# luoyetx/JDA

Measured on AMD Instinct MI355X. Metric: candidate windows/sec, 640x480 batch (jdaDetect hot path); FDDB images/sec in config.fddb_images_per_s, higher is better.
Workload: dtype f32

## Files before the change

jda_amd/csrc/finish_common.h:

```cpp
#pragma once
#include "kernels_common.h"

namespace jda {

namespace {

template <typename Real>
struct Stp { Real scale, r00, r01, r10, r11; };

template <typename Real>
__device__ __forceinline__ void stp_apply(const Stp<Real>& p, Real x, Real y, Real* x2, Real* y2) {
  *x2 = p.scale * (p.r00 * x + p.r01 * y);
  *y2 = p.scale * (p.r10 * x + p.r11 * y);
}

__device__ __forceinline__ Stp<double> stp_calc(const double* s1, const double* __restrict__ s2, int L,
                                                double* t1, double* t2) {
  double x1c = 0., y1c = 0., x2c = 0., y2c = 0.;
  for (int i = 0; i < L; i++) { x1c += s1[2 * i]; y1c += s1[2 * i + 1]; x2c += s2[2 * i]; y2c += s2[2 * i + 1]; }
  x1c /= (double)L; y1c /= (double)L; x2c /= (double)L; y2c /= (double)L;
  for (int i = 0; i < L; i++) {
    t1[2 * i] = s1[2 * i] - x1c; t1[2 * i + 1] = s1[2 * i + 1] - y1c;
    t2[2 * i] = s2[2 * i] - x2c; t2[2 * i + 1] = s2[2 * i + 1] - y2c;
  }
// ... 97 lines not shown
      const double r = sqrt(2.0);
      v1->ox = (int)((double)x / r); v1->oy = (int)((double)y / r); v1->pw = (int)((double)wn / r);
      v2->ox = x / 2; v2->oy = y / 2; v2->pw = wn / 2;
    }
  }
}

__device__ __forceinline__ void load_window_tile(const uint8_t* __restrict__ wbase, int W, int win, uint8_t* tile,
                                                 int tpitch, int lane, int nthreads = 64, const Bc& bc = Bc()) {
  const int dpr = tpitch >> 2;
  const float inv = 1.0f / (float)dpr;
  const int total = win * dpr;
  uint32_t* t32 = (uint32_t*)tile;
  for (int idx = lane; idx < total; idx += nthreads) {
    const int y = (int)(((float)idx + 0.5f) * inv);
    const int j = idx - y * dpr;
    const uint8_t* p = wbase + (size_t)y * W + 4 * j;
    const unsigned sft = (unsigned)((uintptr_t)p & 3u);
    const uint32_t* q = (const uint32_t*)(p - sft);
#ifdef JDA_BOUNDS_CHECK
    if ((long long)(uintptr_t)q + 4 <= bc.lo || (long long)(uintptr_t)q >= bc.hi) jda_bc_fail(kBcWindowTileLoad, __LINE__);
    if ((int)sft + min(4, win - 4 * j) > 4 && ((long long)(uintptr_t)(q + 1) + 4 <= bc.lo || (long long)(uintptr_t)(q + 1) >= bc.hi)) jda_bc_fail(kBcWindowTileLoad, __LINE__);
    JDA_BC(Bc(0, (long long)tpitch * win), (long long)idx * 4, 4, kBcWindowTileLoad);
#endif
    const uint32_t lo = q[0];
    uint32_t hi = 0;
    if ((int)sft + min(4, win - 4 * j) > 4) hi = q[1];
    t32[idx] = __builtin_amdgcn_alignbyte(hi, lo, sft);
  }
}

}

template <typename DL, int G, bool MULTI, bool ST, bool TILE = false>
__device__ __forceinline__ void walk_carts(const NodeOff<typename DL::Real>* __restrict__ stage_off,
                                           const uint2* __restrict__ stage_meta, int K, const int* k,
                                           int depth, int node_n, const typename DL::Real* sh, int win,
                                           const View& v0, const View& v1, const View& v2,
                                           const Stp<typename DL::Real>& stp, bool apply_st, int* leaf,
                                           const uint8_t* tile = nullptr, int tpitch = 0,
                                           const typename DL::Node* __restrict__ stage_deep = nullptr, int split = 1 << 20) {
  int node[G];
#pragma unroll
  for (int g = 0; g < G; g++) node[g] = 0;
  const int levels = depth - 1;
  const int shallow = min(levels, split);
  for (int d = 0; d < shallow; d++) {
    const unsigned first = (1u << d) - 1u, lvl = (unsigned)K * first - first;
    typename DL::Node nd[G];
#pragma unroll
    for (int g = 0; g < G; g++) {
      const unsigned o = lvl + ((unsigned)k[g] << d) + (unsigned)node[g];
      const NodeOff<typename DL::Real> f = stage_off[o];
      const uint2 mt = stage_meta[o];
      nd[g].o1x = f.o1x; nd[g].o1y = f.o1y; nd[g].o2x = f.o2x; nd[g].o2y = f.o2y;
      nd[g].lm1x2 = (int)(mt.x & 0x7fffu); nd[g].lm2x2 = (int)((mt.x >> 15) & 0x7fffu); nd[g].scale = (int)(mt.x >> 30);
      nd[g].th = (int)mt.y;
    }
    int feat[G];
#pragma unroll
    for (int g = 0; g < G; g++) feat[g] = node_feature<DL, MULTI, ST, TILE>(nd[g], sh, win, v0, v1, v2, stp, apply_st, tile, tpitch);
#pragma unroll
    for (int g = 0; g < G; g++) node[g] = 2 * node[g] + (feat[g] <= nd[g].th ? 1 : 2);
  }
  for (int d = shallow; d < levels; d++) {
    typename DL::Node nd[G];
#pragma unroll
    for (int g = 0; g < G; g++)
      nd[g] = stage_deep[lm_deep_index((unsigned)k[g], (unsigned)d, (unsigned)node[g], (unsigned)levels, (unsigned)split)];
    int feat[G];
#pragma unroll
    for (int g = 0; g < G; g++) feat[g] = node_feature<DL, MULTI, ST, TILE>(nd[g], sh, win, v0, v1, v2, stp, apply_st, tile, tpitch);
#pragma unroll
    for (int g = 0; g < G; g++) node[g] = 2 * node[g] + (feat[g] <= nd[g].th ? 1 : 2);
  }
#pragma unroll
  for (int g = 0; g < G; g++) leaf[g] = node[g] - node_n;
}

template <int G, bool TILE>
__device__ __forceinline__ void walk_carts_s0(const S0Node* __restrict__ tbl, int K, const int* k, int depth, int node_n,
                                              const uint8_t* __restrict__ pix, int pitch, int* leaf, const Bc& bc = Bc()) {
  int node[G];
#pragma unroll
  for (int g = 0; g < G; g++) node[g] = 0;
  for (int d = 0; d < depth - 1; d++) {
    const unsigned first = (1u << d) - 1u, lvl = (unsigned)K * first - first;
    S0Node r[G];
#pragma unroll
    for (int g = 0; g < G; g++) r[g] = tbl[lvl + ((unsigned)k[g] << d) + (unsigned)node[g]];
    int pa[G], pb[G];
#pragma unroll
    for (int g = 0; g < G; g++) {
      const unsigned p1 = r[g].lo & 0x3fffffu, p2 = __builtin_amdgcn_alignbit(r[g].hi, r[g].lo, 22) & 0x3fffffu;
#ifdef JDA_BOUNDS_CHECK
      if (TILE) { JDA_BC(bc, __umul24(p1 >> 11, (unsigned)pitch) + (p1 & 0x7ffu), 1, kBcFinishTile); JDA_BC(bc, __umul24(p2 >> 11, (unsigned)pitch) + (p2 & 0x7ffu), 1, kBcFinishTile); }
      else { JDA_BC_ADDR(bc, pix + __umul24(p1 >> 11, (unsigned)pitch) + (p1 & 0x7ffu), 1, kBcFinishPix); JDA_BC_ADDR(bc, pix + __umul24(p2 >> 11, (unsigned)pitch) + (p2 & 0x7ffu), 1, kBcFinishPix); }
#endif
      pa[g] = pix[__umul24(p1 >> 11, (unsigned)pitch) + (p1 & 0x7ffu)];
      pb[g] = pix[__umul24(p2 >> 11, (unsigned)pitch) + (p2 & 0x7ffu)];
    }
#pragma unroll
    for (int g = 0; g < G; g++) node[g] = 2 * node[g] + (pa[g] - pb[g] <= (int)((r[g].hi >> 12) & 0x3ffu) - 256 ? 1 : 2);
  }
#pragma unroll
  for (int g = 0; g < G; g++) leaf[g] = node[g] - node_n;
}


}
```

jda_amd/csrc/host.h:

```cpp
#pragma once
#include <hip/hip_runtime_api.h>

#include <algorithm>
#include <atomic>
#include <chrono>
#include <cmath>
#include <cstdio>
#include <cstdlib>
#include <cstring>
#include <condition_variable>
#include <exception>
#include <functional>
#include <memory>
#include <map>
#include <mutex>
#include <numeric>
#include <new>
#include <stdexcept>
#include <string>
#include <thread>
#include <tuple>
#include <vector>

#include "../../include/jda.h"
// ... 35 lines not shown
  catch (...) {}
  try { fail(std::string(fn) + ": " + what); }
  catch (...) { std::fprintf(stderr, "libjda: %s: %s\n", fn, what); }
  if (sync_device) { (void)hipDeviceSynchronize(); (void)hipGetLastError(); }
}
#define JDA_ABI_CATCH(ret) catch (...) { jda::abi_exception(__func__, false); return ret; }
#define JDA_ABI_CATCH_SYNC(ret) catch (...) { jda::abi_exception(__func__, true); return ret; }
#define JDA_ABI_CATCH_VOID catch (...) { jda::abi_exception(__func__, false); }

constexpr int kLdsGranule = 1280, kLdsGranules = 128;
inline int lds_wgs_per_cu(long long lds_bytes) { return lds_bytes <= 0 ? kLdsGranules : (int)(kLdsGranules / ((lds_bytes + kLdsGranule - 1) / kLdsGranule)); }
inline int lds_bytes_for_wgs(int wgs_per_cu) { return (kLdsGranules / std::max(1, wgs_per_cu)) * kLdsGranule; }

inline long long env_ll(const char* name, long long dflt) {
  const char* v = std::getenv(name);
  return v && *v ? std::atoll(v) : dflt;
}

#define JDA_KNOBS(X)                                                                                   \
  X(handoff, "JDA_HANDOFF", 128)             \
  X(no_fast_scan, "JDA_NO_FAST_SCAN", 0)                                                               \
  X(plan_cache, "JDA_PLAN_CACHE", 64)                                 \
  X(dense, "JDA_DENSE", 1)                                                \
  X(merge_blocks, "JDA_MERGE_BLOCKS", 2048)  \
  X(side_small, "JDA_SIDE_SMALL", 1)                                                                   \
  X(side_stream, "JDA_SIDE_STREAM", 1)                                                                 \
  X(wide_max, "JDA_WIDE_MAX", 1024)          \
  X(wide_conc, "JDA_WIDE_CONC", 1)           \
  X(h2d_stream, "JDA_H2D_STREAM", 1)         \
  X(h2d_min_bytes, "JDA_H2D_MIN_BYTES", 8 << 20)  \
  X(kernel_d2h, "JDA_KERNEL_D2H", 1)         \
  X(filter0, "JDA_FILTER0", 1)               \
  X(fin_carry, "JDA_FIN_CARRY", 1)           \
  X(predict, "JDA_PREDICT", 1)               \
  X(debug_times, "JDA_DEBUG_TIMES", 0)                                                                 \
  X(test_wpf_scale, "JDA_TEST_WPF_SCALE", 1)              \
  X(test_throw, "JDA_TEST_THROW", 0)         \
  X(lanes, "JDA_LANES", 2)                                 \
  X(lanes_min_windows, "JDA_LANES_MIN_WINDOWS", 2000000)                                               \
  X(workspace_mb, "JDA_WORKSPACE_MB", 24 * 1024)                                                       \
  X(ws_bound, "JDA_WS_BOUND", 1)             \
  X(ws_factor_pct, "JDA_WS_FACTOR_PCT", 400)  \
  X(ws_min_entries, "JDA_WS_MIN_ENTRIES", 65536)  \
  X(ragged_chunk_windows, "JDA_RAGGED_CHUNK_WINDOWS", 4000000)  \
  X(ragged_chunk_windows_cpp, "JDA_RAGGED_CHUNK_WINDOWS_CPP", 8000000)  \
  X(mine_chunk_windows, "JDA_MINE_CHUNK_WINDOWS", 4194304)  \
  X(lbf_lds_kb, "JDA_LBF_LDS_KB", 160)       \
  X(ragged_chunk_min_windows, "JDA_RAGGED_CHUNK_MIN_WINDOWS", 1500000)  \
  X(ragged_split, "JDA_RAGGED_SPLIT", 3)     \
  X(ragged_single_windows, "JDA_RAGGED_SINGLE_WINDOWS", 5000000)  \
  X(hwq_place, "JDA_HWQ_PLACE", 1)           \
  X(max_lanes, "JDA_MAX_LANES", 16)          \
  X(lane_idle_calls, "JDA_LANE_IDLE_CALLS", 256)  \
  X(device_post, "JDA_DEVICE_POST", 1)       \
  X(device_post_min_frames, "JDA_DEVICE_POST_MIN_FRAMES", 16)  \
  X(w_pad, "JDA_W_PAD", 1)                   \
  X(lm_deep, "JDA_LM_DEEP", 1)               \
  X(w_stream_mb, "JDA_W_STREAM_MB", 8)       \
  X(scan_p, "JDA_SCAN_P", 1)                 \
  X(scan_p_ragged, "JDA_SCAN_P_RAGGED", 1)   \
  X(scan_p_block, "JDA_SCAN_P_BLOCK", 768)                               \
  X(scan_p_slots, "JDA_SCAN_P_SLOTS", 5)     \
  X(scan_p_b0, "JDA_SCAN_P_B0", 32)                \
  X(scan_p_b1, "JDA_SCAN_P_B1", 64)                                                                    \
  X(scan_p_b2, "JDA_SCAN_P_B2", 0)                                                                     \
  X(scan_p_b3, "JDA_SCAN_P_B3", 0)                                                                     \
// ... 455 lines not shown
```

jda_amd/csrc/k_finish.hip:

```cpp
#include "finish_common.h"

#ifndef FIN_ROW_BATCH
#define FIN_ROW_BATCH 0
#endif

namespace jda {


template <typename DL, bool TRACE, int kG, bool MULTI, bool ST, bool STREAM = false>
__global__ __launch_bounds__(64) void k_finish(const DevPlan* __restrict__ plan, DevModelT<typename DL::Real> m,
                                               WorkT<typename DL::Real> w, int multi_i, float inv_sqrt2,
                                               int t_begin, int t_end, int apply_th, typename DL::Real final_th,
                                               const S0Node* __restrict__ s0_table, int tile_win, int survivors) {
  using Real = typename DL::Real;
  constexpr bool kCpp = sizeof(Real) == 8;
  extern __shared__ __attribute__((aligned(16))) unsigned char lds[];
  const int lane = threadIdx.x;
  const int T = m.T, K = m.K, node_n = m.node_n, leaf_n = m.leaf_n, dim = m.dim, w_pitch = m.w_pitch;
  const int dim_pad = (dim + 1) & ~1;
  Real* sh = (Real*)lds;
  uint32_t* lbf = (uint32_t*)(sh + dim_pad);
  int* stage_cnt = (int*)(lbf + ((K + 3) & ~3));
  Real* st_tmp = (Real*)(stage_cnt + kMaxStages);
  uint8_t* tile = lds + (((size_t)((unsigned char*)(st_tmp + (ST ? 2 * dim_pad + 8 : 0)) - lds) + 15) & ~(size_t)15);
  constexpr bool multi = MULTI;
  (void)multi_i;
  if (lane < kMaxStages) stage_cnt[lane] = 0;
  const bool from_scan = t_begin == 0 && !survivors;
  const unsigned n = (unsigned)min(w.counters[from_scan ? kCntTail : kCntMid], (unsigned long long)(from_scan ? w.cap_q : w.cap_m));
  unsigned long long carts_acc = 0;

#ifdef JDA_SCAN_TIMING
  unsigned long long stamps[15];
  int n_stamp = 0;
  int dbg_win = 0;
#define JDA_FSTAMP() do { if (n_stamp < 15) stamps[n_stamp++] = __builtin_amdgcn_s_memtime(); } while (0)
#else
#define JDA_FSTAMP() do { } while (0)
#endif
  for (unsigned i = blockIdx.x; i < n; i += gridDim.x) {
    JDA_FSTAMP();
    const uint32_t gid = from_scan ? w.q_gid[i] : w.m_gid[i];
// ... 33 lines not shown

    bool alive = true;
    int carts_n = 0;
    for (int t = t_begin; t < t_end; t++) {
      const NodeOff<Real>* n_off = (const NodeOff<Real>*)m.lm_off + (size_t)t * K * node_n;
      const uint2* n_meta = m.lm_meta + (size_t)t * K * node_n;
      const int n_split = m.lm_split;
      const typename DL::Node* n_deep = (const typename DL::Node*)m.lm_deep + (size_t)t * K * (node_n - ((1 << min(n_split, m.D - 1)) - 1));
      const Real* leaf_tab = m.leaf + (size_t)t * K * leaf_n;
      const Real* cth = m.cth + (size_t)t * K;
      const Real* cmean = m.cmean + (size_t)t * K;
      const Real* cstd = m.cstd + (size_t)t * K;
      const uint8_t* cnorm = m.cnorm + (size_t)t * K;
      const int kbeg = t == 0 ? min(kstart, K) : 0;
      const bool carried = t == 0 && kc < K;
      const int k_first = carried ? kc : kbeg & ~63;
      Stp<Real> stp;
      stp.scale = 1; stp.r00 = 1; stp.r01 = 0; stp.r10 = 0; stp.r11 = 1;
      if constexpr (ST) {
        const bool stale = t == m.similarity - 2;
        if (lane == 0 && (!stale || t == t_begin)) {
          Stp<double> p;
          p.scale = 1.; p.r00 = 1.; p.r01 = 0.; p.r10 = 0.; p.r11 = 1.;
          if (!stale) p = stp_calc((const double*)sh, (const double*)m.mean_shape_raw, m.L, (double*)st_tmp, (double*)st_tmp + dim_pad);
          double* o = (double*)st_tmp + 2 * dim_pad;
          o[0] = p.scale; o[1] = p.r00; o[2] = p.r01; o[3] = p.r10; o[4] = p.r11;
        }
        __syncthreads();
        const Real* o = st_tmp + 2 * dim_pad;
        stp.scale = o[0]; stp.r00 = o[1]; stp.r01 = o[2]; stp.r10 = o[3]; stp.r11 = o[4];
      }
      const bool apply_st = ST && t > 0;

      for (int k0 = carried ? K : k_first; k0 < K && alive; k0 += 64 * kG) {
        int kk[kG], lf[kG], nrm[kG];
        Real ls[kG], thk[kG], mk[kG], sk[kG];
#pragma unroll
        for (int g = 0; g < kG; g++) kk[g] = min(k0 + g * 64 + lane, K - 1);
        if (t == 0 && s0_tbl && use_tile) walk_carts_s0<kG, true>(s0_tbl, K, kk, m.D, node_n, tile, tpitch, lf, Bc(0, (long long)tpitch * win));
        else if (t == 0 && s0_tbl) walk_carts_s0<kG, false>(s0_tbl, K, kk, m.D, node_n, wbase, v0.w, lf, v0.bc);
        else if (!MULTI && use_tile) walk_carts<DL, kG, MULTI, ST, true>(n_off, n_meta, K, kk, m.D, node_n, sh, win, v0, v1, v2, stp, apply_st, lf, tile, tpitch, n_deep, n_split);
        else walk_carts<DL, kG, MULTI, ST>(n_off, n_meta, K, kk, m.D, node_n, sh, win, v0, v1, v2, stp, apply_st, lf, nullptr, 0, n_deep, n_split);
#pragma unroll
        for (int g = 0; g < kG; g++) {
          const int k = k0 + g * 64 + lane;
          ls[g] = 0; thk[g] = 0; mk[g] = 0; sk[g] = 1; nrm[g] = 0;
          if (k < K) {
            lbf[k] = (uint32_t)(k * leaf_n + lf[g]) * (uint32_t)w_pitch;
            ls[g] = leaf_tab[(unsigned)(k * leaf_n + lf[g])];
            thk[g] = cth[k];
            nrm[g] = cnorm[k];
            if (nrm[g]) { mk[g] = cmean[k]; sk[g] = cstd[k]; }
          }
        }
#pragma unroll
        for (int g = 0; g < kG; g++) {
          const int kg = k0 + g * 64;
          if (kg >= K || !alive) break;
          const unsigned long long normmask = __ballot(nrm[g] != 0);
          const int jr = replay_scores<Real, TRACE>(score, hash, ls[g], thk[g], mk[g], sk[g], normmask, lf[g],
                                                    max(0, kbeg - kg), min(64, K - kg));
          if (jr >= 0) { alive = false; carts_n = t * K + kg + jr + 1; }
        }
        if (t == t_begin) JDA_FSTAMP();
      }
      if (t != t_begin) JDA_FSTAMP();
      if (!alive) break;
      if (carried) {
        const int bits = carry_bits(leaf_n);
        const uint32_t word = w.m_leaf[(size_t)i * 64 + lane];
        for (int k = kc + lane; k < K; k += 64)
          lbf[k] = (uint32_t)(k * leaf_n + carry_unpack(word, bits, k >> 6)) * (uint32_t)w_pitch;
        JDA_FSTAMP();
      }
      for (int k0 = 0; k0 < k_first; k0 += 128) {
        int kk[2], lf[2];
        kk[0] = min(k0 + lane, k_first - 1); kk[1] = min(k0 + 64 + lane, k_first - 1);
        if (t == 0 && s0_tbl && use_tile) walk_carts_s0<2, true>(s0_tbl, K, kk, m.D, node_n, tile, tpitch, lf, Bc(0, (long long)tpitch * win));
        else if (t == 0 && s0_tbl) walk_carts_s0<2, false>(s0_tbl, K, kk, m.D, node_n, wbase, v0.w, lf, v0.bc);
        else if (!MULTI && use_tile) walk_carts<DL, 2, MULTI, ST, true>(n_off, n_meta, K, kk, m.D, node_n, sh, win, v0, v1, v2, stp, apply_st, lf, tile, tpitch, n_deep, n_split);
        else walk_carts<DL, 2, MULTI, ST>(n_off, n_meta, K, kk, m.D, node_n, sh, win, v0, v1, v2, stp, apply_st, lf, nullptr, 0, n_deep, n_split);
        if (k0 + lane < k_first) lbf[k0 + lane] = (uint32_t)((k0 + lane) * leaf_n + lf[0]) * (uint32_t)w_pitch;
        if (k0 + 64 + lane < k_first) lbf[k0 + 64 + lane] = (uint32_t)((k0 + 64 + lane) * leaf_n + lf[1]) * (uint32_t)w_pitch;
      }
      __syncthreads();
      if (t == t_begin) JDA_FSTAMP();
      const Real* wt = m.w_rows + (size_t)t * K * leaf_n * w_pitch;
      for (int d = lane; d < dim; d += 64) {
        Real acc = kCpp ? (Real)0 : sh[d];
        const Real* col = wt + d;
        int k = 0;
#ifdef JDA_EXP_NOREG
        k = K;
#endif
        constexpr int RB = FIN_ROW_BATCH > 0 ? FIN_ROW_BATCH : (kCpp ? 32 : 64);
        for (; k + RB <= K; k += RB) {
          Real r[RB];
#pragma unroll
          for (int u = 0; u < RB; u++) { JDA_BC(Bc(0, (long long)K * leaf_n * w_pitch), (long long)lbf[k + u] + d, 1, kBcWRow); r[u] = STREAM ? __builtin_nontemporal_load(col + lbf[k + u]) : col[lbf[k + u]]; }
#pragma unroll
          for (int u = 0; u < RB; u++) acc = acc + r[u];
        }
        for (; k < K; k++) { JDA_BC(Bc(0, (long long)K * leaf_n * w_pitch), (long long)lbf[k] + d, 1, kBcWRow); acc = acc + col[lbf[k]]; }
        if (kCpp) {
          const Real other = __shfl_xor(acc, 1);
          acc = (d & 1) ? stp.scale * (stp.r10 * other + stp.r11 * acc) : stp.scale * (stp.r00 * acc + stp.r01 * other);
          acc = sh[d] + acc;
        }
        sh[d] = acc;
      }
      __syncthreads();
      JDA_FSTAMP();
      if (lane == 0) stage_cnt[t] += 1;
    }

    if (!alive || t_end == T) {
      if (alive) carts_n = T * K;
      carts_acc += (unsigned long long)carts_n;
      if (TRACE) {
        if (lane == 0) { w.tr_carts[gid] = carts_n; w.tr_score[gid] = score; w.tr_hash[gid] = hash; }
        for (int d = lane; d < dim; d += 64) w.tr_shape[(size_t)gid * dim + d] = sh[d];
      }
      if (alive && !(apply_th && score < final_th)) {
        unsigned o = 0;
        if (lane == 0) o = (unsigned)atomicAdd(&w.counters[kCntOut], 1ull);
        o = (unsigned)__shfl((int)o, 0);
        if (o < w.cap_m) {
          if (lane == 0) { w.out_gid[o] = gid; w.out_score[o] = score; }
          for (int d = lane; d < dim; d += 64) w.out_shape[(size_t)o * dim + d] = sh[d];
        }
      }
    } else {
      unsigned o = 0;
      if (lane == 0) o = (unsigned)atomicAdd(&w.counters[kCntMid], 1ull);
      o = (unsigned)__shfl((int)o, 0);
      if (o < w.cap_m) {
        if (lane == 0) { w.m_gid[o] = gid; w.m_score[o] = score; w.m_xy[o] = xy; w.m_wf[o] = wf; if (TRACE) w.m_hash[o] = hash; }
        for (int d = lane; d < dim; d += 64) w.m_shape[(size_t)o * dim + d] = sh[d];
      }
    }
  }
#ifdef JDA_SCAN_TIMING
  JDA_FSTAMP();
// ... 134 lines not shown
        if (TRACE && lane == 0) { w.tr_carts[gid[u]] = rej[u] + 1; w.tr_score[gid[u]] = score[u]; w.tr_hash[gid[u]] = hash[u]; }
      } else {
        unsigned o = 0;
        if (lane == 0) o = (unsigned)atomicAdd(&w.counters[kCntMid], 1ull);
        o = (unsigned)__shfl((int)o, 0);
        if (o < w.cap_m && lane == 0) {
          w.m_gid[o] = gid[u]; w.m_score[o] = score[u]; w.m_xy[o] = xy[u]; w.m_wf[o] = wf[u];
          if (TRACE) w.m_hash[o] = hash[u];
        }
        if (carry && o < w.cap_m) {
          const bool room = o < w.cap_l && kbeg[u] < K;
          if (room) w.m_leaf[(size_t)o * 64 + lane] = packed[u];
          if (lane == 0) w.m_k0[o] = room ? (uint32_t)(kbeg[u] & ~63) : (uint32_t)K;
        }
      }
    }
  }
  if (lane == 0 && carts_acc) atomicAdd(shard_counter(w.counters, kCntCarts), carts_acc);
}

template <typename Real>
hipError_t launch_filter0(bool trace, const DevPlan* d_plan, const DevModelT<Real>& m, const WorkT<Real>& w, long long n_hint,
                          const S0Node* s0_table, hipStream_t stream) {
  using DL = typename std::conditional<sizeof(Real) == 4, DialectC, DialectCPP>::type;
  const unsigned blocks = (unsigned)std::max<long long>(1, std::min<long long>((n_hint + 7) / 8, 1 << 20));
  if (trace) hipLaunchKernelGGL((k_filter0<DL, true>), dim3(blocks), dim3(256), 0, stream, d_plan, m, w, s0_table);
  else hipLaunchKernelGGL((k_filter0<DL, false>), dim3(blocks), dim3(256), 0, stream, d_plan, m, w, s0_table);
  return hipGetLastError();
}
template hipError_t launch_filter0<float>(bool, const DevPlan*, const DevModelT<float>&, const WorkT<float>&, long long, const S0Node*, hipStream_t);
template hipError_t launch_filter0<double>(bool, const DevPlan*, const DevModelT<double>&, const WorkT<double>&, long long, const S0Node*, hipStream_t);

namespace {
template <typename DL>
hipError_t launch_finish_impl(bool trace, int t_begin, int t_end, bool apply_th, typename DL::Real th,
                              const DevPlan* d_plan, const DevModelT<typename DL::Real>& m,
                              const WorkT<typename DL::Real>& w, int groups, long long n_hint, const S0Node* s0_table,
                              int tile_win, bool survivors, hipStream_t stream) {
  using Real = typename DL::Real;
  const int dim_pad = (m.dim + 1) & ~1;
  const bool st = sizeof(Real) == 8 && m.similarity != 0;
  const int multi = (w.half != nullptr) ? 1 : 0;
  if (multi) tile_win = 0;
  const size_t base = (size_t)dim_pad * sizeof(Real) + (size_t)((m.K + 3) & ~3) * 4 + kMaxStages * sizeof(int) +
                      (st ? (2 * (size_t)dim_pad + 8) * sizeof(Real) : 0);
  if (tile_win < 0) {
    tile_win = 0;
    for (int tw = 16; tw <= 255; tw++)
      if (base + (size_t)tw * ((tw + 3) & ~3) + 16 <= kFinishLdsPerGroup) tile_win = tw;
  }
  const size_t tile_bytes = tile_win > 0 ? (size_t)tile_win * ((tile_win + 3) & ~3) + 16 : 0;
  const size_t lds = base + tile_bytes;
  const float r = 1.f / sqrtf(2.f);
  unsigned blocks = t_begin == 0 && !survivors ? w.cap_q : w.cap_m;
  if (blocks > 256u * 64u) blocks = 256u * 64u;
  if (n_hint >= 0) blocks = (unsigned)std::min<long long>(n_hint, 1 << 20);
  if (blocks == 0) return hipSuccess;
  auto go = [&](auto kern) {
    if (lds > 48 * 1024) (void)hipFuncSetAttribute((const void*)kern, hipFuncAttributeMaxDynamicSharedMemorySize, (int)lds);
    hipLaunchKernelGGL(kern, dim3(blocks), dim3(64), lds, stream, d_plan, m, w, multi, r, t_begin, t_end,
                       apply_th ? 1 : 0, th, s0_table, tile_win, survivors ? 1 : 0);
  };
  auto pick = [&](auto trace_tag, auto multi_tag, auto st_tag) {
    constexpr bool TR = decltype(trace_tag)::value, MU = decltype(multi_tag)::value;
    constexpr bool STT = decltype(st_tag)::value && sizeof(Real) == 8;
    if constexpr (!TR && !MU && !STT) {
      if (m.w_stream) {
        if (groups >= 4) go(k_finish<DL, false, 4, false, false, true>);
        else if (groups == 3) go(k_finish<DL, false, 3, false, false, true>);
        else if (groups >= 2) go(k_finish<DL, false, 2, false, false, true>);
        else go(k_finish<DL, false, 1, false, false, true>);
        return;
      }
    }
    if (groups >= 4) go(k_finish<DL, TR, 4, MU, STT>);
    else if (groups == 3) go(k_finish<DL, TR, 3, MU, STT>);
    else if (groups >= 2) go(k_finish<DL, TR, 2, MU, STT>);
    else go(k_finish<DL, TR, 1, MU, STT>);
  };
  auto pick_m = [&](auto trace_tag, auto st_tag) {
    if (multi) pick(trace_tag, std::true_type{}, st_tag); else pick(trace_tag, std::false_type{}, st_tag);
  };
  if (st) { if (trace) pick_m(std::true_type{}, std::true_type{}); else pick_m(std::false_type{}, std::true_type{}); }
  else { if (trace) pick_m(std::true_type{}, std::false_type{}); else pick_m(std::false_type{}, std::false_type{}); }
  return hipGetLastError();
}
}

template <>
hipError_t launch_finish<float>(bool trace, int t_begin, int t_end, bool apply_final_th, float final_th,
                                const DevPlan* d_plan, const DevModelT<float>& m, const WorkT<float>& w,
                                int groups, long long n_hint, const S0Node* s0_table, int tile_win, hipStream_t stream,
                                bool survivors) {
  return launch_finish_impl<DialectC>(trace, t_begin, t_end, apply_final_th, final_th, d_plan, m, w, groups, n_hint, s0_table, tile_win, survivors, stream);
}
template <>
hipError_t launch_finish<double>(bool trace, int t_begin, int t_end, bool apply_final_th, double final_th,
                                 const DevPlan* d_plan, const DevModelT<double>& m, const WorkT<double>& w,
                                 int groups, long long n_hint, const S0Node* s0_table, int tile_win, hipStream_t stream,
                                 bool survivors) {
  return launch_finish_impl<DialectCPP>(trace, t_begin, t_end, apply_final_th, final_th, d_plan, m, w, groups, n_hint, s0_table, tile_win, survivors, stream);
}


JDA_BC_READER(k_finish)

}
```

jda_amd/csrc/kernels.h:

```cpp
#pragma once
#include <hip/hip_runtime_api.h>

#include <cstddef>
#include <cstdint>

namespace jda {

constexpr int kMaxLevels = 64;
constexpr int kMaxStages = 16;

struct DevLevel {
  int win, step, nx, ny;
  int base;
  int tiled;
  int tw, th;
  int tiles_x, tiles_y;
  int pitch;
  int s0_table;
};

struct DevPlan {
  int n_levels;
  int width, height;
  int windows;
// ... 173 lines not shown
                       const WorkT<Real>& w, hipStream_t stream, int lv_lo = 0, int lv_hi = kMaxLevels);

template <typename Real>
hipError_t launch_scan_ragged(int mode, int block, bool trace, int handoff, int cp_max, int opts, const DevPlan* d_plan,
                              const DevModelT<Real>& m, const S0Node* table, const WorkT<Real>& w, int pix_bytes,
                              int blk_base, int blk_n, hipStream_t stream);

constexpr int kPScanMaxBuckets = 6;
struct PScanCfg {
  int nb;
  int bound[kPScanMaxBuckets + 1];
  int lg[kPScanMaxBuckets];
  int slots, slot_bytes, opts;
  int bound_last;
  int any_norm;
  int tw_magic;
  int ring_cap[kPScanMaxBuckets], ring_off[kPScanMaxBuckets], ring_items;
  int th, tiles_y;
  int dyn_slot;
  int to_mid;
};
void scan_p_ring_caps(PScanCfg* cfg, int waves);
size_t scan_p_lds_bytes(const PScanCfg& cfg, int carts, int node_n, int leaf_n, int waves);
hipError_t launch_scan_persistent(int level, const PScanCfg& cfg, int block, int grid_max, const DevPlan* d_plan,
                                  const DevPlan& h_plan, const DevModelT<float>& m, const S0Node* table,
                                  const WorkT<float>& w, hipStream_t stream, int rag_blk_base = 0, int rag_blk_n = -1);

hipError_t launch_repack(const uint8_t* raw, uint8_t* dst, const RagImg* imgs, int n, int max_h, int pitch, hipStream_t stream);

template <typename Real>
hipError_t launch_finish(bool trace, int t_begin, int t_end, bool apply_final_th, Real final_th,
                         const DevPlan* d_plan, const DevModelT<Real>& m, const WorkT<Real>& w,
                         int groups, long long n_hint, const S0Node* s0_table, int tile_win, hipStream_t stream,
                         bool survivors = false);

template <typename Real>
hipError_t launch_filter0(bool trace, const DevPlan* d_plan, const DevModelT<Real>& m, const WorkT<Real>& w, long long n_hint,
                          const S0Node* s0_table, hipStream_t stream);
constexpr size_t kFinishLdsPerGroup = 7680;

bool finish_wide_ok(int dim, int K, int leaf_n, int real_bytes, bool multi, bool similarity);
template <typename Real>
hipError_t launch_finish_wide(bool trace, bool apply_final_th, Real final_th, const DevPlan* d_plan,
                              const DevModelT<Real>& m, const WorkT<Real>& w, long long n_hint, const S0Node* s0_table,
                              hipStream_t stream, bool conc = true);

template <typename Real>
hipError_t launch_stage(bool trace, int level, int t, bool apply_final_th, Real final_th, const DevPlan* d_plan,
                        const DevPlan& h_plan, const DevModelT<Real>& m, const WorkT<Real>& w, int pix_cap,
                        int lds_max, hipStream_t stream);
size_t stage_lds_bytes(int dim, int node_n, int leaf_n, int real_bytes);

hipError_t launch_copy_out(const void* const* src, void* const* dst, const size_t* bytes, int n, hipStream_t stream);

struct PostOut {
  int* n; int* first; int* bb; float* score; float* shape; int* flag;
  unsigned long long* cursor;
  unsigned cap_rows;
};
hipError_t launch_post(const DevPlan* d_plan, const WorkT<float>& w, int dim, int n_frames, bool do_nms, float overlap,
                       const PostOut& o, hipStream_t stream, const uint32_t* rag_gid = nullptr, const RagImg* rag_img = nullptr);

template <typename Real>
hipError_t launch_trace_fill(const DevModelT<Real>& m, const WorkT<Real>& w, unsigned n_windows,
                             hipStream_t stream);


// ... 58 lines not shown
```

jda_amd/csrc/pass.h:

```cpp
#pragma once
#include "host.h"

namespace jda {

inline int scan_p_base_cfg(const Cascador* c, PScanCfg* cfg, int* block, int* wgs) {
  const Knobs& kn = c->kn;
  const int K = std::min(c->hm.K, (int)(kn.scan_p_handoff > 0 ? kn.scan_p_handoff : kn.handoff));
  const long long bs[5] = {kn.scan_p_b0, kn.scan_p_b1, kn.scan_p_b2, kn.scan_p_b3, kn.scan_p_b4};
  int digits[kPScanMaxBuckets] = {6, 6, 6, 6, 6, 6}, nd = 0;
  { long long v = std::max<long long>(0, kn.scan_p_lg); int tmp[16]; int n = 0; while (v > 0 && n < 16) { tmp[n++] = (int)(v % 10); v /= 10; }
    for (int i = n - 1; i >= 0 && nd < kPScanMaxBuckets; i--) digits[nd++] = tmp[i]; }
  int last = 0;
  for (int i = 0; i < 5 && cfg->nb < kPScanMaxBuckets; i++) {
    const int b = (int)bs[i];
    if (b <= last || b >= K) continue;
    cfg->bound[cfg->nb] = b;
    const int d = digits[cfg->nb];
    cfg->lg[cfg->nb] = ((d == 4 || d == 5 || d == 7 || d == 8 || d == 9) && c->hm.leaf_n() <= 256) || d == 2 || d == 3 ? d : 6;
    cfg->nb++;
    last = b;
  }
  cfg->bound[cfg->nb] = K;
  cfg->bound_last = K;
  cfg->any_norm = stage0_any_norm(c->hm, K, true) ? 1 : 0;
// ... 379 lines not shown
      JDA_HIP(hipStreamWaitEvent(ln->side, ln->ev_side[0], 0));
    }
    auto issue = [&](const RaggedChunk::Launch& l, hipStream_t s, bool try_persistent) -> bool {
      if (try_persistent && l.mode == 1 && l.level >= 0 && scan_persistent(l.level, s, &l)) { rs->scan_launches++; my_scan_launches++; return true; }
      JDA_HIP(launch_scan_ragged<Real>(l.mode, l.block, false, handoff, cp_max, opts, pe->dp, m, pe->table, w, l.pix_bytes,
                                       l.blk_base, l.blk_n, s));
      rs->scan_launches++; my_scan_launches++;
      return true;
    };
    if (fork_glb) {
      for (const RaggedChunk::Launch& l : ch.launches)
        if (l.mode == 2) { if (!issue(l, ln->side, false)) return false; side_pending = true; }
    }
    for (const RaggedChunk::Launch& l : ch.launches) {
      if (l.mode == 2 && fork_glb) continue;
      if (fork_glb && kn().ragged_side == 2 && l.mode != 2) {
        if (l.mode == 1 && l.level >= 0 && scan_persistent(l.level, st, &l)) { rs->scan_launches++; my_scan_launches++; continue; }
        if (!issue(l, ln->side, false)) return false;
        continue;
      }
      if (!issue(l, st, true)) return false;
    }
    if (side_pending) JDA_HIP(hipEventRecord(ln->ev_side[1], ln->side));
    if (side_pending) JDA_HIP(hipStreamWaitEvent(st, ln->ev_side[1], 0));
    if (timed) JDA_HIP(hipEventRecord(ev[2], st));
    return issue_rest();
  }

  bool launch_finishers(long long n_grid) {
    const int T = hm().T;
    const int gm = kn().fin_gm > 0 ? (int)kn().fin_gm : stage_groups();
    const int g2 = kn().fin_g2 > 0 ? (int)kn().fin_g2 : stage_groups();
    n_grid = std::max<long long>(n_grid, 1);
    WorkT<Real> wc = w;
    if (!carry_ok()) wc.m_leaf = nullptr;
    if (mid_direct) {
      const long long nmid = pred_mid >= 0 ? (long long)(pred_mid * (double)windows() * 1.25) + 64 : 0;
      const long long wg2 = std::min<long long>((long long)cap_m, std::max<long long>(std::max<long long>(2048, n_grid / std::max<long long>(1, kn().fin_grid_div)), nmid));
      JDA_HIP(launch_filter0<Real>(want_trace(), pe->dp, model(), wc, n_grid, s0_tbl(), st));
      JDA_HIP(launch_finish<Real>(want_trace(), 0, T, apply_th, th, pe->dp, model(), wc, g2, wg2, s0_tbl(), (int)kn().fin_tile, st, true));
      finished = true;
      return true;
    }
    if (n_grid <= kn().wide_max && busy_lanes <= kn().wide_busy_max && finish_wide_ok(hm().dim(), hm().K, hm().leaf_n(), (int)sizeof(Real), multi, Sel<Real>::dialect == JDA_DIALECT_CPP && c->similarity)) {
      JDA_HIP(launch_finish_wide<Real>(want_trace(), apply_th, th, pe->dp, model(), w, n_grid, s0_tbl(), st, kn().wide_conc != 0));
      finished = true;
      return true;
    }
    const bool st_snapshot = sizeof(Real) == 8 && c->similarity && hm().hdr_stage >= 0 && hm().hdr_stage < T;
    if (T == 1 || n_grid <= kn().finish_merge || st_snapshot) {
      JDA_HIP(launch_finish<Real>(want_trace(), 0, T, apply_th, th, pe->dp, model(), w, gm, n_grid, s0_tbl(), (int)kn().fin_tile, st));
      finished = true;
      return true;
    }
    const long long wg2 = std::min<long long>(n_grid, std::max<long long>(2048, n_grid / std::max<long long>(1, kn().fin_grid_div)));
    if (filter0_ok()) {
      JDA_HIP(launch_filter0<Real>(want_trace(), pe->dp, model(), wc, n_grid, s0_tbl(), st));
      JDA_HIP(launch_finish<Real>(want_trace(), 0, T, apply_th, th, pe->dp, model(), wc, g2, wg2, s0_tbl(), (int)kn().fin_tile, st, true));
      finished = true;
      return true;
    }
    JDA_HIP(launch_finish<Real>(want_trace(), 0, 1, apply_th, th, pe->dp, model(), w, (int)kn().fin_g1, n_grid, s0_tbl(), (int)kn().fin_tile1, st));
    JDA_HIP(launch_finish<Real>(want_trace(), 1, T, apply_th, th, pe->dp, model(), w, g2, wg2, nullptr, (int)kn().fin_tile, st));
    finished = true;
    return true;
  }

  bool after_tail() {
    if (finished) return true;
    JDA_HIP(hipStreamSynchronize(st));
    const unsigned long long true_tail = h_cnt[0], true_mid = mid_direct ? h_cnt[kCntMid - kCntTail] : 0ull;
    n_tail = (long long)std::min<unsigned long long>(true_tail, cap_q);
    const long long n_alive = (long long)(true_tail + true_mid);
    int pix_cap, lds_max;
    const double dense_frac = (double)kn().dense_pct / 100.0;
    if (dense_ok(&pix_cap, &lds_max) && (double)n_alive >= dense_frac * (double)windows() && n_alive > 4096) {
      { std::lock_guard<std::mutex> lk(c->mu); pe->dense_hint = true; }
      if (!rag) {
        dense = true; finished = true;
        if (!grow_for_dense() || !clear_counters()) return false;
        return run_dense();
      }
    }
    if (true_tail > cap_q || true_mid > cap_m) return recover_overflow(true_tail, true_mid, 0);
    return launch_finishers(n_tail);
  }

  bool after_mid() { return true; }

  bool issue_counters() {
    if (counters_issued) return true;
    counters_issued = true;
    if (timed) JDA_HIP(hipEventRecord(ev[3], st));
    if (kn().kernel_d2h) {
      const void* src[1] = {w.counters}; void* dst[1] = {h_cnt};
      const size_t nb[1] = {sizeof(unsigned long long) * kCntShards * kCntStride};
// ... 238 lines not shown
```

Before: 7.424 billion.

## Overlap deferred score replay with next tree walk and weight-row loads

The finish kernel now defers each 64-lane group's score replay and runs it inside the next batch of cart walks and inside the global-row accumulation loop, right after the loads are issued, so replay arithmetic hides memory latency. A Fill callback hook is threaded into walk_carts and walk_carts_s0, and a host-side check falls back to the plain kernel if the overlapped variant would lose occupancy by register count. Early exit on rejection can now abort the row accumulation, and the dim loop is padded to full waves. The cost is extra registers and added control-flow complexity.

```diff
diff --git a/jda_amd/csrc/finish_common.h b/jda_amd/csrc/finish_common.h
--- a/jda_amd/csrc/finish_common.h
+++ b/jda_amd/csrc/finish_common.h
@@ -153,14 +153,17 @@
 
 }
 
-template <typename DL, int G, bool MULTI, bool ST, bool TILE = false>
+struct NoFill { __device__ __forceinline__ void operator()() const {} };
+
+template <typename DL, int G, bool MULTI, bool ST, bool TILE = false, typename Fill = NoFill>
 __device__ __forceinline__ void walk_carts(const NodeOff<typename DL::Real>* __restrict__ stage_off,
                                            const uint2* __restrict__ stage_meta, int K, const int* k,
                                            int depth, int node_n, const typename DL::Real* sh, int win,
                                            const View& v0, const View& v1, const View& v2,
                                            const Stp<typename DL::Real>& stp, bool apply_st, int* leaf,
                                            const uint8_t* tile = nullptr, int tpitch = 0,
-                                           const typename DL::Node* __restrict__ stage_deep = nullptr, int split = 1 << 20) {
+                                           const typename DL::Node* __restrict__ stage_deep = nullptr, int split = 1 << 20,
+                                           Fill fill = Fill()) {
   int node[G];
 #pragma unroll
   for (int g = 0; g < G; g++) node[g] = 0;
@@ -169,11 +172,19 @@
   for (int d = 0; d < shallow; d++) {
     const unsigned first = (1u << d) - 1u, lvl = (unsigned)K * first - first;
     typename DL::Node nd[G];
+    NodeOff<typename DL::Real> fs[G];
+    uint2 mts[G];
 #pragma unroll
     for (int g = 0; g < G; g++) {
       const unsigned o = lvl + ((unsigned)k[g] << d) + (unsigned)node[g];
-      const NodeOff<typename DL::Real> f = stage_off[o];
-      const uint2 mt = stage_meta[o];
+      fs[g] = stage_off[o];
+      mts[g] = stage_meta[o];
+    }
+    fill();
+#pragma unroll
+    for (int g = 0; g < G; g++) {
+      const NodeOff<typename DL::Real> f = fs[g];
+      const uint2 mt = mts[g];
       nd[g].o1x = f.o1x; nd[g].o1y = f.o1y; nd[g].o2x = f.o2x; nd[g].o2y = f.o2y;
       nd[g].lm1x2 = (int)(mt.x & 0x7fffu); nd[g].lm2x2 = (int)((mt.x >> 15) & 0x7fffu); nd[g].scale = (int)(mt.x >> 30);
       nd[g].th = (int)mt.y;
@@ -189,6 +200,7 @@
 #pragma unroll
     for (int g = 0; g < G; g++)
       nd[g] = stage_deep[lm_deep_index((unsigned)k[g], (unsigned)d, (unsigned)node[g], (unsigned)levels, (unsigned)split)];
+    fill();
     int feat[G];
 #pragma unroll
     for (int g = 0; g < G; g++) feat[g] = node_feature<DL, MULTI, ST, TILE>(nd[g], sh, win, v0, v1, v2, stp, apply_st, tile, tpitch);
@@ -199,9 +211,10 @@
   for (int g = 0; g < G; g++) leaf[g] = node[g] - node_n;
 }
 
-template <int G, bool TILE>
+template <int G, bool TILE, typename Fill = NoFill>
 __device__ __forceinline__ void walk_carts_s0(const S0Node* __restrict__ tbl, int K, const int* k, int depth, int node_n,
-                                              const uint8_t* __restrict__ pix, int pitch, int* leaf, const Bc& bc = Bc()) {
+                                              const uint8_t* __restrict__ pix, int pitch, int* leaf, const Bc& bc = Bc(),
+                                              Fill fill = Fill()) {
   int node[G];
 #pragma unroll
   for (int g = 0; g < G; g++) node[g] = 0;
@@ -210,6 +223,7 @@
     S0Node r[G];
 #pragma unroll
     for (int g = 0; g < G; g++) r[g] = tbl[lvl + ((unsigned)k[g] << d) + (unsigned)node[g]];
+    fill();
     int pa[G], pb[G];
 #pragma unroll
     for (int g = 0; g < G; g++) {
diff --git a/jda_amd/csrc/host.h b/jda_amd/csrc/host.h
--- a/jda_amd/csrc/host.h
+++ b/jda_amd/csrc/host.h
@@ -91,6 +91,7 @@
   X(kernel_d2h, "JDA_KERNEL_D2H", 1)         \
   X(filter0, "JDA_FILTER0", 1)               \
   X(fin_carry, "JDA_FIN_CARRY", 1)           \
+  X(fin_overlap, "JDA_FIN_OVERLAP", 1)       \
   X(predict, "JDA_PREDICT", 1)               \
   X(debug_times, "JDA_DEBUG_TIMES", 0)                                                                 \
   X(test_wpf_scale, "JDA_TEST_WPF_SCALE", 1)              \
diff --git a/jda_amd/csrc/k_finish.hip b/jda_amd/csrc/k_finish.hip
--- a/jda_amd/csrc/k_finish.hip
+++ b/jda_amd/csrc/k_finish.hip
@@ -1,4 +1,7 @@
 #include "finish_common.h"
+
+#include <map>
+#include <mutex>
 
 #ifndef FIN_ROW_BATCH
 #define FIN_ROW_BATCH 0
@@ -7,7 +10,7 @@
 namespace jda {
 
 
-template <typename DL, bool TRACE, int kG, bool MULTI, bool ST, bool STREAM = false>
+template <typename DL, bool TRACE, int kG, bool MULTI, bool ST, bool STREAM = false, bool OVL = false>
 __global__ __launch_bounds__(64) void k_finish(const DevPlan* __restrict__ plan, DevModelT<typename DL::Real> m,
                                                WorkT<typename DL::Real> w, int multi_i, float inv_sqrt2,
                                                int t_begin, int t_end, int apply_th, typename DL::Real final_th,
@@ -107,35 +110,73 @@
       }
       const bool apply_st = ST && t > 0;
 
+      Real p_ls[kG], p_th[kG];
+      int p_lf[kG], p_nr[kG];
+      int p_n = 0, p_kg = 0;
+      auto replay_front = [&]() {
+        Real mk = 0, sk = 1;
+        const unsigned long long normmask = __ballot(p_nr[0] != 0);
+        if (normmask != 0ull) {
+          const int k = p_kg + lane;
+          if (p_nr[0] != 0) { mk = cmean[k]; sk = cstd[k]; }
+        }
+#ifdef JDA_EXP_NOREPLAY
+        int jr = -1;
+#else
+        const int jr = replay_scores<Real, TRACE>(score, hash, p_ls[0], p_th[0], mk, sk, normmask, TRACE ? p_lf[0] : 0,
+                                                  max(0, kbeg - p_kg), min(64, K - p_kg));
+#endif
+        if (jr >= 0) { alive = false; carts_n = t * K + p_kg + jr + 1; p_n = 0; return; }
+#pragma unroll
+        for (int g = 0; g + 1 < kG; g++) {
+          p_ls[g] = p_ls[g + 1]; p_th[g] = p_th[g + 1]; p_nr[g] = p_nr[g + 1];
+          if (TRACE) p_lf[g] = p_lf[g + 1];
+        }
+        p_kg += 64; p_n -= 1;
+      };
+      auto fill = [&]() { if (OVL && p_n > 0 && alive) replay_front(); };
       for (int k0 = carried ? K : k_first; k0 < K && alive; k0 += 64 * kG) {
         int kk[kG], lf[kG], nrm[kG];
-        Real ls[kG], thk[kG], mk[kG], sk[kG];
+        Real mk[kG], sk[kG];
 #pragma unroll
         for (int g = 0; g < kG; g++) kk[g] = min(k0 + g * 64 + lane, K - 1);
-        if (t == 0 && s0_tbl && use_tile) walk_carts_s0<kG, true>(s0_tbl, K, kk, m.D, node_n, tile, tpitch, lf, Bc(0, (long long)tpitch * win));
-        else if (t == 0 && s0_tbl) walk_carts_s0<kG, false>(s0_tbl, K, kk, m.D, node_n, wbase, v0.w, lf, v0.bc);
-        else if (!MULTI && use_tile) walk_carts<DL, kG, MULTI, ST, true>(n_off, n_meta, K, kk, m.D, node_n, sh, win, v0, v1, v2, stp, apply_st, lf, tile, tpitch, n_deep, n_split);
-        else walk_carts<DL, kG, MULTI, ST>(n_off, n_meta, K, kk, m.D, node_n, sh, win, v0, v1, v2, stp, apply_st, lf, nullptr, 0, n_deep, n_split);
+        if (t == 0 && s0_tbl && use_tile) walk_carts_s0<kG, true>(s0_tbl, K, kk, m.D, node_n, tile, tpitch, lf, Bc(0, (long long)tpitch * win), fill);
+        else if (t == 0 && s0_tbl) walk_carts_s0<kG, false>(s0_tbl, K, kk, m.D, node_n, wbase, v0.w, lf, v0.bc, fill);
+        else if (!MULTI && use_tile) walk_carts<DL, kG, MULTI, ST, true>(n_off, n_meta, K, kk, m.D, node_n, sh, win, v0, v1, v2, stp, apply_st, lf, tile, tpitch, n_deep, n_split, fill);
+        else walk_carts<DL, kG, MULTI, ST>(n_off, n_meta, K, kk, m.D, node_n, sh, win, v0, v1, v2, stp, apply_st, lf, nullptr, 0, n_deep, n_split, fill);
+        if constexpr (OVL) {
+          while (p_n > 0 && alive) replay_front();
+          if (!alive) break;
+        }
 #pragma unroll
         for (int g = 0; g < kG; g++) {
           const int k = k0 + g * 64 + lane;
-          ls[g] = 0; thk[g] = 0; mk[g] = 0; sk[g] = 1; nrm[g] = 0;
+          p_ls[g] = 0; p_th[g] = 0; mk[g] = 0; sk[g] = 1; nrm[g] = 0;
           if (k < K) {
             lbf[k] = (uint32_t)(k * leaf_n + lf[g]) * (uint32_t)w_pitch;
-            ls[g] = leaf_tab[(unsigned)(k * leaf_n + lf[g])];
-            thk[g] = cth[k];
+            p_ls[g] = leaf_tab[(unsigned)(k * leaf_n + lf[g])];
+            p_th[g] = cth[k];
             nrm[g] = cnorm[k];
-            if (nrm[g]) { mk[g] = cmean[k]; sk[g] = cstd[k]; }
+            if (!OVL && nrm[g]) { mk[g] = cmean[k]; sk[g] = cstd[k]; }
           }
         }
-#pragma unroll
-        for (int g = 0; g < kG; g++) {
-          const int kg = k0 + g * 64;
-          if (kg >= K || !alive) break;
-          const unsigned long long normmask = __ballot(nrm[g] != 0);
-          const int jr = replay_scores<Real, TRACE>(score, hash, ls[g], thk[g], mk[g], sk[g], normmask, lf[g],
-                                                    max(0, kbeg - kg), min(64, K - kg));
-          if (jr >= 0) { alive = false; carts_n = t * K + kg + jr + 1; }
+        if constexpr (OVL) {
+#pragma unroll
+          for (int g = 0; g < kG; g++) { p_nr[g] = nrm[g]; if (TRACE) p_lf[g] = lf[g]; }
+          p_kg = k0; p_n = min(kG, (K - k0 + 63) >> 6);
+        } else {
+#pragma unroll
+          for (int g = 0; g < kG; g++) {
+            const int kg = k0 + g * 64;
+            if (kg >= K || !alive) break;
+#ifdef JDA_EXP_NOREPLAY
+            break;
+#endif
+            const unsigned long long normmask = __ballot(nrm[g] != 0);
+            const int jr = replay_scores<Real, TRACE>(score, hash, p_ls[g], p_th[g], mk[g], sk[g], normmask, lf[g],
+                                                      max(0, kbeg - kg), min(64, K - kg));
+            if (jr >= 0) { alive = false; carts_n = t * K + kg + jr + 1; }
+          }
         }
         if (t == t_begin) JDA_FSTAMP();
       }
@@ -148,20 +189,22 @@
           lbf[k] = (uint32_t)(k * leaf_n + carry_unpack(word, bits, k >> 6)) * (uint32_t)w_pitch;
         JDA_FSTAMP();
       }
-      for (int k0 = 0; k0 < k_first; k0 += 128) {
+      for (int k0 = 0; k0 < k_first && alive; k0 += 128) {
         int kk[2], lf[2];
         kk[0] = min(k0 + lane, k_first - 1); kk[1] = min(k0 + 64 + lane, k_first - 1);
-        if (t == 0 && s0_tbl && use_tile) walk_carts_s0<2, true>(s0_tbl, K, kk, m.D, node_n, tile, tpitch, lf, Bc(0, (long long)tpitch * win));
-        else if (t == 0 && s0_tbl) walk_carts_s0<2, false>(s0_tbl, K, kk, m.D, node_n, wbase, v0.w, lf, v0.bc);
-        else if (!MULTI && use_tile) walk_carts<DL, 2, MULTI, ST, true>(n_off, n_meta, K, kk, m.D, node_n, sh, win, v0, v1, v2, stp, apply_st, lf, tile, tpitch, n_deep, n_split);
-        else walk_carts<DL, 2, MULTI, ST>(n_off, n_meta, K, kk, m.D, node_n, sh, win, v0, v1, v2, stp, apply_st, lf, nullptr, 0, n_deep, n_split);
+        if (t == 0 && s0_tbl && use_tile) walk_carts_s0<2, true>(s0_tbl, K, kk, m.D, node_n, tile, tpitch, lf, Bc(0, (long long)tpitch * win), fill);
+        else if (t == 0 && s0_tbl) walk_carts_s0<2, false>(s0_tbl, K, kk, m.D, node_n, wbase, v0.w, lf, v0.bc, fill);
+        else if (!MULTI && use_tile) walk_carts<DL, 2, MULTI, ST, true>(n_off, n_meta, K, kk, m.D, node_n, sh, win, v0, v1, v2, stp, apply_st, lf, tile, tpitch, n_deep, n_split, fill);
+        else walk_carts<DL, 2, MULTI, ST>(n_off, n_meta, K, kk, m.D, node_n, sh, win, v0, v1, v2, stp, apply_st, lf, nullptr, 0, n_deep, n_split, fill);
         if (k0 + lane < k_first) lbf[k0 + lane] = (uint32_t)((k0 + lane) * leaf_n + lf[0]) * (uint32_t)w_pitch;
         if (k0 + 64 + lane < k_first) lbf[k0 + 64 + lane] = (uint32_t)((k0 + 64 + lane) * leaf_n + lf[1]) * (uint32_t)w_pitch;
       }
       __syncthreads();
       if (t == t_begin) JDA_FSTAMP();
       const Real* wt = m.w_rows + (size_t)t * K * leaf_n * w_pitch;
-      for (int d = lane; d < dim; d += 64) {
+      for (int d0 = 0; d0 < dim; d0 += 64) {
+        if (!OVL && d0 + lane >= dim) continue;
+        const int d = OVL ? min(d0 + lane, dim - 1) : d0 + lane;
         Real acc = kCpp ? (Real)0 : sh[d];
         const Real* col = wt + d;
         int k = 0;
@@ -169,12 +212,24 @@
         k = K;
 #endif
         constexpr int RB = FIN_ROW_BATCH > 0 ? FIN_ROW_BATCH : (kCpp ? 32 : 64);
-        for (; k + RB <= K; k += RB) {
-          Real r[RB];
-#pragma unroll
-          for (int u = 0; u < RB; u++) { JDA_BC(Bc(0, (long long)K * leaf_n * w_pitch), (long long)lbf[k + u] + d, 1, kBcWRow); r[u] = STREAM ? __builtin_nontemporal_load(col + lbf[k + u]) : col[lbf[k + u]]; }
-#pragma unroll
-          for (int u = 0; u < RB; u++) acc = acc + r[u];
+        constexpr int RBF = kCpp ? RB : RB * 3 / 4;
+        auto rows = [&](auto n_tag, auto fill_tag) {
+          constexpr int N = decltype(n_tag)::value;
+          Real r[N];
+#pragma unroll
+          for (int u = 0; u < N; u++) { JDA_BC(Bc(0, (long long)K * leaf_n * w_pitch), (long long)lbf[k + u] + d, 1, kBcWRow); r[u] = STREAM ? __builtin_nontemporal_load(col + lbf[k + u]) : col[lbf[k + u]]; }
+          if constexpr (decltype(fill_tag)::value) replay_front();
+#pragma unroll
+          for (int u = 0; u < N; u++) acc = acc + r[u];
+          k += N;
+        };
+        if constexpr (OVL) {
+          while (p_n > 0 && alive && k + RBF <= K) rows(std::integral_constant<int, RBF>{}, std::true_type{});
+        }
+        while (k + RB <= K && (!OVL || alive)) rows(std::integral_constant<int, RB>{}, std::false_type{});
+        if constexpr (OVL) {
+          while (p_n > 0 && alive) replay_front();
+          if (!alive) break;
         }
         for (; k < K; k++) { JDA_BC(Bc(0, (long long)K * leaf_n * w_pitch), (long long)lbf[k] + d, 1, kBcWRow); acc = acc + col[lbf[k]]; }
         if (kCpp) {
@@ -182,8 +237,9 @@
           acc = (d & 1) ? stp.scale * (stp.r10 * other + stp.r11 * acc) : stp.scale * (stp.r00 * acc + stp.r01 * other);
           acc = sh[d] + acc;
         }
-        sh[d] = acc;
-      }
+        if (!OVL || d0 + lane < dim) sh[d] = acc;
+      }
+      if (OVL && !alive) break;
       __syncthreads();
       JDA_FSTAMP();
       if (lane == 0) stage_cnt[t] += 1;
@@ -384,11 +440,25 @@
 template hipError_t launch_filter0<double>(bool, const DevPlan*, const DevModelT<double>&, const WorkT<double>&, long long, const S0Node*, hipStream_t);
 
 namespace {
+int finish_waves(const void* kern) {
+  static std::mutex mu;
+  static std::map<const void*, int> known;
+  std::lock_guard<std::mutex> lock(mu);
+  auto it = known.find(kern);
+  if (it != known.end()) return it->second;
+  hipFuncAttributes a{};
+  int waves = 4;
+  if (hipFuncGetAttributes(&a, kern) == hipSuccess && a.numRegs > 0) waves = std::min(4, 512 / ((a.numRegs + 7) & ~7));
+  else (void)hipGetLastError();
+  known[kern] = waves;
+  return waves;
+}
+
 template <typename DL>
 hipError_t launch_finish_impl(bool trace, int t_begin, int t_end, bool apply_th, typename DL::Real th,
                               const DevPlan* d_plan, const DevModelT<typename DL::Real>& m,
                               const WorkT<typename DL::Real>& w, int groups, long long n_hint, const S0Node* s0_table,
-                              int tile_win, bool survivors, hipStream_t stream) {
+                              int tile_win, bool survivors, bool overlap, hipStream_t stream) {
   using Real = typename DL::Real;
   const int dim_pad = (m.dim + 1) & ~1;
   const bool st = sizeof(Real) == 8 && m.similarity != 0;
@@ -413,28 +483,37 @@
     hipLaunchKernelGGL(kern, dim3(blocks), dim3(64), lds, stream, d_plan, m, w, multi, r, t_begin, t_end,
                        apply_th ? 1 : 0, th, s0_table, tile_win, survivors ? 1 : 0);
   };
-  auto pick = [&](auto trace_tag, auto multi_tag, auto st_tag) {
+  auto pick = [&](auto trace_tag, auto multi_tag, auto st_tag, auto ovl_tag) {
     constexpr bool TR = decltype(trace_tag)::value, MU = decltype(multi_tag)::value;
     constexpr bool STT = decltype(st_tag)::value && sizeof(Real) == 8;
+    constexpr bool OV = decltype(ovl_tag)::value;
+    auto go2 = [&](auto kern, auto plain) {
+      if (OV && !TR && finish_waves((const void*)kern) < finish_waves((const void*)plain)) go(plain); else go(kern);
+    };
     if constexpr (!TR && !MU && !STT) {
       if (m.w_stream) {
-        if (groups >= 4) go(k_finish<DL, false, 4, false, false, true>);
-        else if (groups == 3) go(k_finish<DL, false, 3, false, false, true>);
-        else if (groups >= 2) go(k_finish<DL, false, 2, false, false, true>);
-        else go(k_finish<DL, false, 1, false, false, true>);
+        if (groups >= 4) go2(k_finish<DL, false, 4, false, false, true, OV>, k_finish<DL, false, 4, false, false, true, false>);
+        else if (groups == 3) go2(k_finish<DL, false, 3, false, false, true, OV>, k_finish<DL, false, 3, false, false, true, false>);
+        else if (groups >= 2) go2(k_finish<DL, false, 2, false, false, true, OV>, k_finish<DL, false, 2, false, false, true, false>);
+        else go2(k_finish<DL, false, 1, false, false, true, OV>, k_finish<DL, false, 1, false, false, true, false>);
         return;
       }
     }
-    if (groups >= 4) go(k_finish<DL, TR, 4, MU, STT>);
-    else if (groups == 3) go(k_finish<DL, TR, 3, MU, STT>);
-    else if (groups >= 2) go(k_finish<DL, TR, 2, MU, STT>);
-    else go(k_finish<DL, TR, 1, MU, STT>);
+    if (groups >= 4) go2(k_finish<DL, TR, 4, MU, STT, false, OV>, k_finish<DL, TR, 4, MU, STT, false, false>);
+    else if (groups == 3) go2(k_finish<DL, TR, 3, MU, STT, false, OV>, k_finish<DL, TR, 3, MU, STT, false, false>);
+    else if (groups >= 2) go2(k_finish<DL, TR, 2, MU, STT, false, OV>, k_finish<DL, TR, 2, MU, STT, false, false>);
+    else go2(k_finish<DL, TR, 1, MU, STT, false, OV>, k_finish<DL, TR, 1, MU, STT, false, false>);
   };
-  auto pick_m = [&](auto trace_tag, auto st_tag) {
-    if (multi) pick(trace_tag, std::true_type{}, st_tag); else pick(trace_tag, std::false_type{}, st_tag);
+  auto pick_m = [&](auto trace_tag, auto st_tag, auto ovl_tag) {
+    if (multi) pick(trace_tag, std::true_type{}, st_tag, ovl_tag); else pick(trace_tag, std::false_type{}, st_tag, ovl_tag);
   };
-  if (st) { if (trace) pick_m(std::true_type{}, std::true_type{}); else pick_m(std::false_type{}, std::true_type{}); }
-  else { if (trace) pick_m(std::true_type{}, std::false_type{}); else pick_m(std::false_type{}, std::false_type{}); }
+  auto pick_t = [&](auto st_tag, auto ovl_tag) {
+    if (trace) pick_m(std::true_type{}, st_tag, ovl_tag); else pick_m(std::false_type{}, st_tag, ovl_tag);
+  };
+  auto pick_s = [&](auto ovl_tag) {
+    if (st) pick_t(std::true_type{}, ovl_tag); else pick_t(std::false_type{}, ovl_tag);
+  };
+  if (overlap) pick_s(std::true_type{}); else pick_s(std::false_type{});
   return hipGetLastError();
 }
 }
@@ -443,15 +522,15 @@
 hipError_t launch_finish<float>(bool trace, int t_begin, int t_end, bool apply_final_th, float final_th,
                                 const DevPlan* d_plan, const DevModelT<float>& m, const WorkT<float>& w,
                                 int groups, long long n_hint, const S0Node* s0_table, int tile_win, hipStream_t stream,
-                                bool survivors) {
-  return launch_finish_impl<DialectC>(trace, t_begin, t_end, apply_final_th, final_th, d_plan, m, w, groups, n_hint, s0_table, tile_win, survivors, stream);
+                                bool survivors, bool overlap) {
+  return launch_finish_impl<DialectC>(trace, t_begin, t_end, apply_final_th, final_th, d_plan, m, w, groups, n_hint, s0_table, tile_win, survivors, overlap, stream);
 }
 template <>
 hipError_t launch_finish<double>(bool trace, int t_begin, int t_end, bool apply_final_th, double final_th,
                                  const DevPlan* d_plan, const DevModelT<double>& m, const WorkT<double>& w,
                                  int groups, long long n_hint, const S0Node* s0_table, int tile_win, hipStream_t stream,
-                                 bool survivors) {
-  return launch_finish_impl<DialectCPP>(trace, t_begin, t_end, apply_final_th, final_th, d_plan, m, w, groups, n_hint, s0_table, tile_win, survivors, stream);
+                                 bool survivors, bool overlap) {
+  return launch_finish_impl<DialectCPP>(trace, t_begin, t_end, apply_final_th, final_th, d_plan, m, w, groups, n_hint, s0_table, tile_win, survivors, overlap, stream);
 }
 
 
diff --git a/jda_amd/csrc/kernels.h b/jda_amd/csrc/kernels.h
--- a/jda_amd/csrc/kernels.h
+++ b/jda_amd/csrc/kernels.h
@@ -229,7 +229,7 @@
 hipError_t launch_finish(bool trace, int t_begin, int t_end, bool apply_final_th, Real final_th,
                          const DevPlan* d_plan, const DevModelT<Real>& m, const WorkT<Real>& w,
                          int groups, long long n_hint, const S0Node* s0_table, int tile_win, hipStream_t stream,
-                         bool survivors = false);
+                         bool survivors = false, bool overlap = true);
 
 template <typename Real>
 hipError_t launch_filter0(bool trace, const DevPlan* d_plan, const DevModelT<Real>& m, const WorkT<Real>& w, long long n_hint,
diff --git a/jda_amd/csrc/pass.h b/jda_amd/csrc/pass.h
--- a/jda_amd/csrc/pass.h
+++ b/jda_amd/csrc/pass.h
@@ -435,13 +435,14 @@
     const int gm = kn().fin_gm > 0 ? (int)kn().fin_gm : stage_groups();
     const int g2 = kn().fin_g2 > 0 ? (int)kn().fin_g2 : stage_groups();
     n_grid = std::max<long long>(n_grid, 1);
+    const bool ovl = kn().fin_overlap != 0;
     WorkT<Real> wc = w;
     if (!carry_ok()) wc.m_leaf = nullptr;
     if (mid_direct) {
       const long long nmid = pred_mid >= 0 ? (long long)(pred_mid * (double)windows() * 1.25) + 64 : 0;
       const long long wg2 = std::min<long long>((long long)cap_m, std::max<long long>(std::max<long long>(2048, n_grid / std::max<long long>(1, kn().fin_grid_div)), nmid));
       JDA_HIP(launch_filter0<Real>(want_trace(), pe->dp, model(), wc, n_grid, s0_tbl(), st));
-      JDA_HIP(launch_finish<Real>(want_trace(), 0, T, apply_th, th, pe->dp, model(), wc, g2, wg2, s0_tbl(), (int)kn().fin_tile, st, true));
+      JDA_HIP(launch_finish<Real>(want_trace(), 0, T, apply_th, th, pe->dp, model(), wc, g2, wg2, s0_tbl(), (int)kn().fin_tile, st, true, ovl));
       finished = true;
       return true;
     }
@@ -452,19 +453,19 @@
     }
     const bool st_snapshot = sizeof(Real) == 8 && c->similarity && hm().hdr_stage >= 0 && hm().hdr_stage < T;
     if (T == 1 || n_grid <= kn().finish_merge || st_snapshot) {
-      JDA_HIP(launch_finish<Real>(want_trace(), 0, T, apply_th, th, pe->dp, model(), w, gm, n_grid, s0_tbl(), (int)kn().fin_tile, st));
+      JDA_HIP(launch_finish<Real>(want_trace(), 0, T, apply_th, th, pe->dp, model(), w, gm, n_grid, s0_tbl(), (int)kn().fin_tile, st, false, ovl));
       finished = true;
       return true;
     }
     const long long wg2 = std::min<long long>(n_grid, std::max<long long>(2048, n_grid / std::max<long long>(1, kn().fin_grid_div)));
     if (filter0_ok()) {
       JDA_HIP(launch_filter0<Real>(want_trace(), pe->dp, model(), wc, n_grid, s0_tbl(), st));
-      JDA_HIP(launch_finish<Real>(want_trace(), 0, T, apply_th, th, pe->dp, model(), wc, g2, wg2, s0_tbl(), (int)kn().fin_tile, st, true));
+      JDA_HIP(launch_finish<Real>(want_trace(), 0, T, apply_th, th, pe->dp, model(), wc, g2, wg2, s0_tbl(), (int)kn().fin_tile, st, true, ovl));
       finished = true;
       return true;
     }
-    JDA_HIP(launch_finish<Real>(want_trace(), 0, 1, apply_th, th, pe->dp, model(), w, (int)kn().fin_g1, n_grid, s0_tbl(), (int)kn().fin_tile1, st));
-    JDA_HIP(launch_finish<Real>(want_trace(), 1, T, apply_th, th, pe->dp, model(), w, g2, wg2, nullptr, (int)kn().fin_tile, st));
+    JDA_HIP(launch_finish<Real>(want_trace(), 0, 1, apply_th, th, pe->dp, model(), w, (int)kn().fin_g1, n_grid, s0_tbl(), (int)kn().fin_tile1, st, false, ovl));
+    JDA_HIP(launch_finish<Real>(want_trace(), 1, T, apply_th, th, pe->dp, model(), w, g2, wg2, nullptr, (int)kn().fin_tile, st, false, ovl));
     finished = true;
     return true;
   }
```

Result: slower. 7.219 billion (-2.8%).
